# OpenBMB/VisRAG

Measured on NVIDIA H100. Metric: page-images encoded/sec, higher is better.
Workload: dtype bf16

## Files before the change

visrag_b200/csrc/gemm.cu:

```cuda
#include "common.h"
#include "gemm.cuh"

namespace vr {

template <bool F16, int BN, int MODE, bool OUT_F32, bool GELU, bool SWAP = false>
static int launch_gemm(const void* A, int64_t lda, const void* B, int64_t ldb, const GemmArgs& g, cudaStream_t stream) {
    using Cfg = GemmCfg<BN>;
    CUtensorMap ta, tb;
    if (int rc = make_tmap_2d(SWAP ? &tb : &ta, A, g.M, g.K, lda, SWAP ? 64 : GEMM_BM, GEMM_BK, 128, !F16)) return rc;
    if (int rc = make_tmap_2d(SWAP ? &ta : &tb, B, g.N, g.K, ldb, SWAP ? GEMM_BM : 64, GEMM_BK, 128, !F16)) return rc;
    auto kern = gemm_wgmma_kernel<F16, BN, MODE, OUT_F32, GELU, SWAP>;
    static unsigned long long attr_set = 0;
    if (first_use_on_device(&attr_set))
        VR_CHECK_CUDA(cudaFuncSetAttribute(kern, cudaFuncAttributeMaxDynamicSharedMemorySize, Cfg::SMEM_BYTES));
    const int tiles = SWAP ? ((g.N + GEMM_BM - 1) / GEMM_BM) * ((g.M + BN - 1) / BN)
                           : ((g.M + GEMM_BM - 1) / GEMM_BM) * ((g.N + BN - 1) / BN);
    const int grid = tiles < num_sms() ? tiles : num_sms();
    kern<<<grid, GEMM_THREADS, Cfg::SMEM_BYTES, stream>>>(ta, tb, g);
    VR_CHECK_CUDA(cudaGetLastError());
    return 0;
}

template <bool F16, int MODE, bool OUT_F32, bool GELU, int CLUSTER, bool LEAN>
static int launch_pingpong(const void* A, int64_t lda, const void* B, int64_t ldb, const GemmArgs& g, bool l2_slices,
                           cudaStream_t stream) {
    CUtensorMap ta, tb;
    if (int rc = make_tmap_2d(&ta, A, g.M, g.K, lda, GEMM_BM, GEMM_BK, 128, !F16)) return rc;
    if (int rc = make_tmap_2d(&tb, B, g.N, g.K, ldb, 64, GEMM_BK, 128, !F16)) return rc;
    auto kern = gemm_pingpong_kernel<F16, MODE, OUT_F32, GELU, CLUSTER, LEAN>;
    cudaLaunchConfig_t cfg = {};
    cudaLaunchAttribute attr[1];
    cfg.blockDim = dim3(GEMM_THREADS);
    cfg.dynamicSmemBytes = GEMM_PP_SMEM_BYTES;
    cfg.stream = stream;
    attr[0].id = cudaLaunchAttributeClusterDimension;
    attr[0].val.clusterDim.x = CLUSTER;
    attr[0].val.clusterDim.y = 1;
    attr[0].val.clusterDim.z = 1;
    cfg.attrs = attr;
    cfg.numAttrs = 1;
    static unsigned long long attr_set = 0;
    static int max_clusters[64] = {};
    const int dev = current_device(), dev_slot = dev >= 0 && dev < 64 ? dev : 0;
    if (first_use_on_device(&attr_set)) {
        VR_CHECK_CUDA(cudaFuncSetAttribute(kern, cudaFuncAttributeMaxDynamicSharedMemorySize, GEMM_PP_SMEM_BYTES));
        int n = num_sms() / CLUSTER;
        if (CLUSTER > 1) {
            cfg.gridDim = dim3(num_sms() / CLUSTER * CLUSTER);
            VR_CHECK_CUDA(cudaOccupancyMaxActiveClusters(&n, kern, &cfg));
        }
        max_clusters[dev_slot] = n;
    }
    const PPSched sch = pp_schedule(g.M, g.N, g.K, CLUSTER, l2_slices);
    VR_REQUIRE(max_clusters[dev_slot] > 0, "vr_gemm: no %d-CTA cluster of the ping-pong kernel fits on this device", CLUSTER);
    const int units = sch.num_units();
    const int clusters = units < max_clusters[dev_slot] ? units : max_clusters[dev_slot];
    cfg.gridDim = dim3(clusters * CLUSTER);
    VR_CHECK_CUDA(cudaLaunchKernelEx(&cfg, kern, ta, tb, g, sch));
    return 0;
}

template <bool F16>
static int check_out_dtype(const vr_gemm_epilogue& e) {
    if (F16) {
        if (e.mode == VR_EPI_LINEAR && e.out_dtype == VR_F32) {
            VR_REQUIRE(!e.act_gelu, "vr_gemm: GELU epilogue writes fp16 only (fp16 operands)");
            return 0;
        }
        if (e.mode == VR_EPI_LINEAR)
            VR_REQUIRE(e.out_dtype == VR_F16, "vr_gemm: with fp16 operands out_dtype must be VR_F16 or VR_F32");
        else
            VR_REQUIRE(e.out_dtype == VR_F16, "vr_gemm: with fp16 operands ROPE / SWIGLU write fp16: out_dtype must be VR_F16");
        return 0;
    }
    if (e.mode != VR_EPI_LINEAR) return 0;
    if (e.out_dtype == VR_F32) {
        VR_REQUIRE(!e.act_gelu, "vr_gemm: GELU epilogue writes bf16 only");
        return 0;
    }
    VR_REQUIRE(e.out_dtype == VR_BF16, "vr_gemm: out_dtype must be VR_BF16 or VR_F32");
    return 0;
}

template <bool F16>
static int dispatch_swapped(const void* A, int64_t lda, const void* B, int64_t ldb, const GemmArgs& g, cudaStream_t s) {
    const vr_gemm_epilogue& e = g.epi;
    VR_REQUIRE(e.mode == VR_EPI_LINEAR, "vr_gemm: block_n=3 (feature-major accumulator) supports LINEAR epilogues only");
    if (int rc = check_out_dtype<F16>(e)) return rc;
    if (e.out_dtype == VR_F32) return launch_gemm<F16, 128, VR_EPI_LINEAR, true, false, true>(A, lda, B, ldb, g, s);
    if (e.act_gelu) return launch_gemm<F16, 128, VR_EPI_LINEAR, false, true, true>(A, lda, B, ldb, g, s);
    return launch_gemm<F16, 128, VR_EPI_LINEAR, false, false, true>(A, lda, B, ldb, g, s);
}

constexpr int PP = 2, PP_MC = 4, PP_NFAST = 5;
template <bool F16, int BN, int MODE, bool OUT_F32, bool GELU, bool LEAN = false>
static int launch_any(const void* A, int64_t lda, const void* B, int64_t ldb, const GemmArgs& g, cudaStream_t s) {
    if constexpr (BN < 0)
        return launch_pingpong<F16, MODE, OUT_F32, GELU, -BN == PP_MC ? 2 : 1, LEAN>(A, lda, B, ldb, g, -BN != PP_NFAST, s);
    else return launch_gemm<F16, BN, MODE, OUT_F32, GELU>(A, lda, B, ldb, g, s);
}

template <bool F16, int BN>
static int dispatch_mode(const void* A, int64_t lda, const void* B, int64_t ldb, const GemmArgs& g, cudaStream_t s) {
    const vr_gemm_epilogue& e = g.epi;
    switch (e.mode) {
        case VR_EPI_LINEAR: {
            if (int rc = check_out_dtype<F16>(e)) return rc;
            if (e.out_dtype == VR_F32) return launch_any<F16, BN, VR_EPI_LINEAR, true, false>(A, lda, B, ldb, g, s);
            const bool lean = BN < 0 && e.bias && e.scale == 1.0f && !e.rowadd && !e.resid;
            if (e.act_gelu)
                return lean ? launch_any<F16, BN, VR_EPI_LINEAR, false, true, true>(A, lda, B, ldb, g, s)
                            : launch_any<F16, BN, VR_EPI_LINEAR, false, true>(A, lda, B, ldb, g, s);
            return lean ? launch_any<F16, BN, VR_EPI_LINEAR, false, false, true>(A, lda, B, ldb, g, s)
                        : launch_any<F16, BN, VR_EPI_LINEAR, false, false>(A, lda, B, ldb, g, s);
        }
        case VR_EPI_ROPE:
            VR_REQUIRE(e.positions && e.rope_cos && e.rope_sin, "vr_gemm: ROPE epilogue needs positions/cos/sin");
            VR_REQUIRE(g.N % 64 == 0 && e.rope_cols % 64 == 0, "vr_gemm: ROPE needs N and rope_cols multiples of 64");
            if (int rc = check_out_dtype<F16>(e)) return rc;
            return launch_any<F16, BN, VR_EPI_ROPE, false, false>(A, lda, B, ldb, g, s);
        case VR_EPI_SWIGLU:
            VR_REQUIRE(g.N % 64 == 0, "vr_gemm: SWIGLU needs N multiple of 64");
            if (int rc = check_out_dtype<F16>(e)) return rc;
            return launch_any<F16, BN, VR_EPI_SWIGLU, false, false>(A, lda, B, ldb, g, s);
        default:
            set_error("vr_gemm: unknown epilogue mode %d", e.mode);
            return 2;
    }
}

template <bool F16>
static int dispatch_block_n(const void* A, int64_t lda, const void* B, int64_t ldb, const GemmArgs& g, int bn, cudaStream_t s) {
    if (bn == PP) return dispatch_mode<F16, -PP>(A, lda, B, ldb, g, s);
    if (bn == PP_MC) return dispatch_mode<F16, -PP_MC>(A, lda, B, ldb, g, s);
    if (bn == PP_NFAST) return dispatch_mode<F16, -PP_NFAST>(A, lda, B, ldb, g, s);
    if (bn == 3) return dispatch_swapped<F16>(A, lda, B, ldb, g, s);
    if (bn == 256) return dispatch_mode<F16, 256>(A, lda, B, ldb, g, s);
    if (bn == 192) return dispatch_mode<F16, 192>(A, lda, B, ldb, g, s);
    if (bn == 128) return dispatch_mode<F16, 128>(A, lda, B, ldb, g, s);
    if (bn == 64) return dispatch_mode<F16, 64>(A, lda, B, ldb, g, s);
    set_error("vr_gemm: block_n must be 0 (auto), 64, 128, 192, 256, 2 / 4 / 5 (ping-pong) or 3 (feature-major accumulator)");
    return 2;
}

}

extern "C" int vr_gemm_tuned(const void* A, int64_t lda, const void* B, int64_t ldb, int32_t ab_dtype, int32_t M,
                             int32_t N, int32_t K, const vr_gemm_epilogue* epi, int32_t block_n, void* stream) {
    using namespace vr;
    VR_REQUIRE(A && B && epi && epi->out, "vr_gemm: null pointer argument");
    VR_REQUIRE(M > 0 && N > 0 && K > 0, "vr_gemm: empty problem M=%d N=%d K=%d", M, N, K);
    VR_REQUIRE(ab_dtype == VR_BF16 || ab_dtype == VR_F16, "vr_gemm: operands must be bf16 or fp16 (got dtype %d)", ab_dtype);
    VR_REQUIRE(N % 8 == 0, "vr_gemm: N=%d must be a multiple of 8", N);
    VR_REQUIRE(K % 8 == 0, "vr_gemm: K=%d must be a multiple of 8 (16-byte TMA rows)", K);
    const int64_t out_cols = epi->mode == VR_EPI_SWIGLU ? N / 2 : N;
    VR_REQUIRE(epi->ldo >= out_cols && epi->ldo % 8 == 0, "vr_gemm: ldo=%lld too small or not a multiple of 8",
               (long long)epi->ldo);
    VR_REQUIRE(epi->mode != VR_EPI_LINEAR || (reinterpret_cast<uintptr_t>(epi->out) & 15) == 0,
               "vr_gemm: a LINEAR out must be 16-byte aligned (out=%p)", epi->out);
    VR_REQUIRE_ALIGNED("vr_gemm", "A", A, 16);
    VR_REQUIRE_ALIGNED("vr_gemm", "B", B, 16);
    VR_REQUIRE_ALIGNED("vr_gemm", "bias", epi->bias, 8);
    VR_REQUIRE_ALIGNED("vr_gemm", "rowadd", epi->rowadd, 8);
    VR_REQUIRE_ALIGNED("vr_gemm", "resid", epi->resid, 8);
    VR_REQUIRE_ALIGNED("vr_gemm", "rope_cos", epi->rope_cos, 8);
    VR_REQUIRE_ALIGNED("vr_gemm", "rope_sin", epi->rope_sin, 8);
    VR_REQUIRE_ALIGNED("vr_gemm", "positions", epi->positions, 4);
    VR_REQUIRE_ALIGNED("vr_gemm", "out", epi->out, 4);
    GemmArgs g;
    g.M = M; g.N = N; g.K = K; g.epi = *epi;
    cudaStream_t s = reinterpret_cast<cudaStream_t>(stream);
    int bn = block_n;
    if (bn == 0) {
        bn = M <= 128 ? 64 : PP_MC;
    }
    return ab_dtype == VR_F16 ? dispatch_block_n<true>(A, lda, B, ldb, g, bn, s) : dispatch_block_n<false>(A, lda, B, ldb, g, bn, s);
}

extern "C" int vr_gemm(const void* A, int64_t lda, const void* B, int64_t ldb, int32_t ab_dtype, int32_t M, int32_t N,
                       int32_t K, const vr_gemm_epilogue* epi, void* stream) {
    return vr_gemm_tuned(A, lda, B, ldb, ab_dtype, M, N, K, epi, 0, stream);
}
```

visrag_b200/csrc/gemm.cuh:

```cuda
#pragma once
#include "ptx.cuh"
#include "../../include/visrag_b200.h"

namespace vr {

constexpr int GEMM_BM = 128;
constexpr int GEMM_BK = 64;
constexpr int GEMM_THREADS = 3 * 128;

template <int BN>
struct GemmCfg {
    static_assert(BN % 64 == 0 && BN <= 256, "tile width: 64, 128, 192 or 256");
    static constexpr int A_BYTES = GEMM_BM * GEMM_BK * 2;
    static constexpr int B_BYTES = BN * GEMM_BK * 2;
    static constexpr int STAGE_BYTES = A_BYTES + B_BYTES;
    static constexpr int STAGES = (192 * 1024) / STAGE_BYTES;
    static constexpr int SMEM_BYTES = STAGES * STAGE_BYTES + 1024  + 256 ;
};

struct GemmArgs {
    int M, N, K;
    vr_gemm_epilogue epi;
};

__device__ __forceinline__ float erf_as(float x) {
    const float ax = fabsf(x);
    float t;
    asm("rcp.approx.ftz.f32 %0, %1;" : "=f"(t) : "f"(fmaf(0.3275911f, ax, 1.0f)));
    float p = fmaf(1.061405429f, t, -1.453152027f);
    p = fmaf(p, t, 1.421413741f);
    p = fmaf(p, t, -0.284496736f);
    p = fmaf(p, t, 0.254829592f);
    p *= t;
    float e;
    asm("ex2.approx.ftz.f32 %0, %1;" : "=f"(e) : "f"(-1.4426950408889634f * ax * ax));
    return copysignf(fmaf(-p, e, 1.0f), x);
}
__device__ __forceinline__ float gelu_erf(float x) { return 0.5f * x * (1.0f + erf_as(x * 0.70710678118654752f)); }

#ifndef VR_GELU_POLY
#define VR_GELU_POLY 1
#endif
#if VR_GELU_POLY
template <int N>
__device__ __forceinline__ void gelu_erf_n(float (&x)[N]) {
    constexpr float R2 = 0.70710678118654752f, ZMAX = 3.2f, A = 2.0f / (ZMAX * ZMAX);
    constexpr float C[11] = {2.982273671e-03f, -7.046153472e-03f, 7.957076705e-03f, -1.521942819e-02f, 3.318292224e-02f,
                             -5.471928813e-02f, 8.062700147e-02f, -1.136467381e-01f, 1.543549678e-01f, -2.173077339e-01f,
                             4.413341836e-01f};
    float z[N], u[N], p[N];
#pragma unroll
    for (int i = 0; i < N; ++i) z[i] = fminf(fmaxf(x[i] * R2, -ZMAX), ZMAX);
#pragma unroll
    for (int i = 0; i < N; ++i) u[i] = fmaf(fmaf(z[i], z[i], 0.0f), A, -1.0f);
#pragma unroll
    for (int i = 0; i < N; ++i) p[i] = fmaf(u[i], C[0], C[1]);
#pragma unroll
    for (int k = 2; k < 11; ++k) {
#pragma unroll
        for (int i = 0; i < N; ++i) p[i] = fmaf(p[i], u[i], C[k]);
    }
#pragma unroll
    for (int i = 0; i < N; ++i) {
        const float r = fmaf(p[i], z[i], 0.0f);
        const float h = 0.5f * x[i];
        x[i] = fmaf(h, r, h);
    }
}
__device__ __forceinline__ void gelu_erf2(float& x0, float& x1) {
    float x[2] = {x0, x1};
    gelu_erf_n(x);
    x0 = x[0];
    x1 = x[1];
}
#else
__device__ __forceinline__ void pk_fma(float& d0, float& d1, float a0, float a1, float b0, float b1, float c0, float c1) {
    d0 = fmaf(a0, b0, c0);
    d1 = fmaf(a1, b1, c1);
}
__device__ __forceinline__ void gelu_erf2(float& x0, float& x1) {
    constexpr float R2 = 0.70710678118654752f;
    const float a0 = fabsf(x0) * R2, a1 = fabsf(x1) * R2;
    float d0, d1, t0, t1, p0, p1, q0, q1, e0, e1, r0, r1;
    pk_fma(d0, d1, a0, a1, 0.3275911f, 0.3275911f, 1.0f, 1.0f);
    asm("rcp.approx.ftz.f32 %0, %1;" : "=f"(t0) : "f"(d0));
    asm("rcp.approx.ftz.f32 %0, %1;" : "=f"(t1) : "f"(d1));
    pk_fma(p0, p1, t0, t1, 1.061405429f, 1.061405429f, -1.453152027f, -1.453152027f);
    pk_fma(p0, p1, p0, p1, t0, t1, 1.421413741f, 1.421413741f);
    pk_fma(p0, p1, p0, p1, t0, t1, -0.284496736f, -0.284496736f);
    pk_fma(p0, p1, p0, p1, t0, t1, 0.254829592f, 0.254829592f);
    pk_fma(p0, p1, p0, p1, t0, t1, 0.0f, 0.0f);
    pk_fma(q0, q1, a0, a1, a0, a1, 0.0f, 0.0f);
    asm("ex2.approx.ftz.f32 %0, %1;" : "=f"(e0) : "f"(q0 * -1.4426950408889634f));
    asm("ex2.approx.ftz.f32 %0, %1;" : "=f"(e1) : "f"(q1 * -1.4426950408889634f));
    pk_fma(r0, r1, p0, p1, -e0, -e1, 1.0f, 1.0f);
    r0 = copysignf(r0, x0);
    r1 = copysignf(r1, x1);
    const float h0 = 0.5f * x0, h1 = 0.5f * x1;
    pk_fma(x0, x1, h0, h1, r0, r1, h0, h1);
}
template <int N>
__device__ __forceinline__ void gelu_erf_n(float (&x)[N]) {
#pragma unroll
    for (int i = 0; i < N; i += 2) gelu_erf2(x[i], x[i + 1]);
}
#endif
__device__ __forceinline__ float silu(float x) {
    float e, r;
    asm("ex2.approx.ftz.f32 %0, %1;" : "=f"(e) : "f"(x * -1.4426950408889634f));
    asm("rcp.approx.ftz.f32 %0, %1;" : "=f"(r) : "f"(1.0f + e));
    return x * r;
}

template <bool F16, bool OUT_F32, bool GELU>
__device__ __forceinline__ void epi_linear2(const GemmArgs& g, int row, int col, float x0, float x1) {
    const vr_gemm_epilogue& e = g.epi;
    if (row >= g.M || col >= g.N) return;
    if (e.bias) {
        const float2 b = *reinterpret_cast<const float2*>(e.bias + col);
        x0 += b.x; x1 += b.y;
    }
    if (GELU) gelu_erf2(x0, x1);
    if (e.scale != 1.0f) { x0 *= e.scale; x1 *= e.scale; }
    if (e.rowadd) {
        const float2 a2 = *reinterpret_cast<const float2*>(e.rowadd + static_cast<long long>(row % e.rowadd_period) * g.N + col);
        x0 += a2.x; x1 += a2.y;
    }
    const long long o = static_cast<long long>(row) * e.ldo + col;
    if (e.resid) {
        const float2 r2 = *reinterpret_cast<const float2*>(e.resid + o);
        x0 += r2.x; x1 += r2.y;
    }
    if (OUT_F32) *reinterpret_cast<float2*>(reinterpret_cast<float*>(e.out) + o) = make_float2(x0, x1);
    else *reinterpret_cast<uint32_t*>(reinterpret_cast<half16_t<F16>*>(e.out) + o) = pack16x2<F16>(x0, x1);
}

template <bool F16, bool OUT_F32, bool GELU>
__device__ __forceinline__ void epi_linear_t(const GemmArgs& g, int tok, int f, float x) {
    const vr_gemm_epilogue& e = g.epi;
    if (tok >= g.M || f >= g.N) return;
    if (e.bias) x += e.bias[f];
    if (GELU) {
        float y = x;
        gelu_erf2(x, y);
    }
    if (e.scale != 1.0f) x *= e.scale;
    if (e.rowadd) x += e.rowadd[static_cast<long long>(tok % e.rowadd_period) * g.N + f];
    const long long o = static_cast<long long>(tok) * e.ldo + f;
    if (e.resid) x += e.resid[o];
    if (OUT_F32) reinterpret_cast<float*>(e.out)[o] = x;
    else reinterpret_cast<half16_t<F16>*>(e.out)[o] = to_half16<F16>(x);
}

template <bool F16>
__device__ __forceinline__ void epi_rope2(const GemmArgs& g, int row, int head0, int c, float lo0, float lo1, float hi0,
                                          float hi1) {
    const vr_gemm_epilogue& e = g.epi;
    if (row >= g.M || head0 >= g.N) return;
    if (head0 < e.rope_cols) {
        const long long pos = e.positions[row];
        const float2 cs = *reinterpret_cast<const float2*>(e.rope_cos + pos * 32 + c);
        const float2 sn = *reinterpret_cast<const float2*>(e.rope_sin + pos * 32 + c);
        const float a0 = lo0, a1 = lo1, b0 = hi0, b1 = hi1;
        lo0 = a0 * cs.x - b0 * sn.x; hi0 = b0 * cs.x + a0 * sn.x;
        lo1 = a1 * cs.y - b1 * sn.y; hi1 = b1 * cs.y + a1 * sn.y;
    }
    half16_t<F16>* o = reinterpret_cast<half16_t<F16>*>(e.out) + static_cast<long long>(row) * e.ldo + head0 + c;
    *reinterpret_cast<uint32_t*>(o) = pack16x2<F16>(lo0, lo1);
    *reinterpret_cast<uint32_t*>(o + 32) = pack16x2<F16>(hi0, hi1);
}

template <bool F16>
__device__ __forceinline__ void epi_swiglu2(const GemmArgs& g, int row, int blk0, int c, float g0, float g1, float u0, float u1) {
    const vr_gemm_epilogue& e = g.epi;
    if (row >= g.M || blk0 >= g.N) return;
    half16_t<F16>* o = reinterpret_cast<half16_t<F16>*>(e.out) + static_cast<long long>(row) * e.ldo + (blk0 >> 1) + c;
    *reinterpret_cast<uint32_t*>(o) = pack16x2<F16>(silu(g0) * u0, silu(g1) * u1);
}

template <bool F16, int BN, int MODE, bool OUT_F32, bool GELU, bool SWAP = false>
__global__ void __launch_bounds__(GEMM_THREADS, 1)
gemm_wgmma_kernel(const __grid_constant__ CUtensorMap tmap_a, const __grid_constant__ CUtensorMap tmap_b, const GemmArgs g) {
    using Cfg = GemmCfg<BN>;
    constexpr int STAGES = Cfg::STAGES;

    extern __shared__ uint8_t smem_raw[];
    uint8_t* smem = reinterpret_cast<uint8_t*>((reinterpret_cast<uintptr_t>(smem_raw) + 1023) & ~uintptr_t(1023));
    uint8_t* smem_a = smem;
    uint8_t* smem_b = smem + STAGES * Cfg::A_BYTES;
    uint64_t* full_bar = reinterpret_cast<uint64_t*>(smem + STAGES * Cfg::STAGE_BYTES);
    uint64_t* empty_bar = full_bar + STAGES;

    const int wg = threadIdx.x >> 7;
    const int warp = (threadIdx.x >> 5) & 3;
    const int lane = threadIdx.x & 31;

    static_assert(!SWAP || MODE == VR_EPI_LINEAR, "feature-major accumulators are implemented for LINEAR epilogues");
    const int tiles_m = ((SWAP ? g.N : g.M) + GEMM_BM - 1) / GEMM_BM;
    const int tiles_n = ((SWAP ? g.M : g.N) + BN - 1) / BN;
    const int num_tiles = tiles_m * tiles_n;
    const int num_kb = (g.K + GEMM_BK - 1) / GEMM_BK;
    auto tile_m0 = [&](int t) { return (SWAP ? t % tiles_m : t / tiles_n) * GEMM_BM; };
    auto tile_n0 = [&](int t) { return (SWAP ? t / tiles_m : t % tiles_n) * BN; };

    if (threadIdx.x == 0) {
        tma_prefetch_desc(&tmap_a);
        tma_prefetch_desc(&tmap_b);
        for (int i = 0; i < STAGES; ++i) {
            mbar_init(&full_bar[i], 1);
            mbar_init(&empty_bar[i], 8);
        }
        fence_mbar_init();
    }
    __syncthreads();

    if (wg == 0) {
        setmaxnreg_dec<40>();
        if (warp == 0 && lane == 0) {
            int stage = 0;
            uint32_t phase = 0;
            for (int t = blockIdx.x; t < num_tiles; t += gridDim.x) {
                const int m0 = tile_m0(t);
                const int n0 = tile_n0(t);
                for (int kb = 0; kb < num_kb; ++kb) {
                    mbar_wait(&empty_bar[stage], phase ^ 1);
                    mbar_expect_tx(&full_bar[stage], Cfg::STAGE_BYTES);
                    tma_load_2d(&tmap_a, &full_bar[stage], smem_a + stage * Cfg::A_BYTES, kb * GEMM_BK, m0);
#pragma unroll
                    for (int h = 0; h < BN / 64; ++h)
                        tma_load_2d(&tmap_b, &full_bar[stage], smem_b + stage * Cfg::B_BYTES + h * (64 * GEMM_BK * 2),
                                    kb * GEMM_BK, n0 + h * 64);
                    if (++stage == STAGES) { stage = 0; phase ^= 1; }
                }
            }
        }
    } else {
        setmaxnreg_inc<232>();
        const int cw = wg - 1;
        const uint64_t desc_hi = make_smem_desc(0, 16, 1024, kLayoutSW128);
        const uint32_t a_lo0 = (smem_u32(smem_a) + cw * (64 * GEMM_BK * 2)) >> 4, b_lo0 = smem_u32(smem_b) >> 4;
        const int g8 = lane >> 2, q = lane & 3;
        int stage = 0;
        uint32_t phase = 0;
        for (int t = blockIdx.x; t < num_tiles; t += gridDim.x) {
            float acc[BN / 2];
            int prev = -1;
            for (int kb = 0; kb < num_kb; ++kb) {
                mbar_wait(&full_bar[stage], phase);
                const uint64_t ad = desc_hi | static_cast<uint64_t>(a_lo0 + stage * (Cfg::A_BYTES >> 4));
                const uint64_t bd = desc_hi | static_cast<uint64_t>(b_lo0 + stage * (Cfg::B_BYTES >> 4));
                wgmma_fence();
#pragma unroll
                for (int kk = 0; kk < 4; ++kk)
                    wgmma_ss<F16, false>(acc, ad + 2 * kk, bd + 2 * kk, (kb | kk) != 0, std::integral_constant<int, BN>());
                wgmma_commit();
                if (prev >= 0) {
                    wgmma_wait<1>();
                    if (lane == 0) mbar_arrive(&empty_bar[prev]);
                }
                prev = stage;
                if (++stage == STAGES) { stage = 0; phase ^= 1; }
            }
            wgmma_wait<0>();
            if (lane == 0) mbar_arrive(&empty_bar[prev]);
            wgmma_touch(acc);

            const int r0 = tile_m0(t) + cw * 64 + warp * 16 + g8;
            const int n0 = tile_n0(t);
            if (MODE == VR_EPI_LINEAR) {
#pragma unroll
                for (int j = 0; j < BN / 8; ++j) {
                    const int c = n0 + j * 8 + q * 2;
                    if (SWAP) {
                        epi_linear_t<F16, OUT_F32, GELU>(g, c, r0, acc[4 * j]);
                        epi_linear_t<F16, OUT_F32, GELU>(g, c + 1, r0, acc[4 * j + 1]);
                        epi_linear_t<F16, OUT_F32, GELU>(g, c, r0 + 8, acc[4 * j + 2]);
                        epi_linear_t<F16, OUT_F32, GELU>(g, c + 1, r0 + 8, acc[4 * j + 3]);
                    } else {
                        epi_linear2<F16, OUT_F32, GELU>(g, r0, c, acc[4 * j], acc[4 * j + 1]);
                        epi_linear2<F16, OUT_F32, GELU>(g, r0 + 8, c, acc[4 * j + 2], acc[4 * j + 3]);
                    }
                }
            } else {
#pragma unroll
                for (int hb = 0; hb < BN / 64; ++hb) {
#pragma unroll
                    for (int j = 0; j < 4; ++j) {
                        const int lo = 4 * (hb * 8 + j), hi = 4 * (hb * 8 + j + 4);
                        const int blk0 = n0 + hb * 64, c = j * 8 + q * 2;
                        if (MODE == VR_EPI_ROPE) {
                            epi_rope2<F16>(g, r0, blk0, c, acc[lo], acc[lo + 1], acc[hi], acc[hi + 1]);
                            epi_rope2<F16>(g, r0 + 8, blk0, c, acc[lo + 2], acc[lo + 3], acc[hi + 2], acc[hi + 3]);
                        } else {
                            epi_swiglu2<F16>(g, r0, blk0, c, acc[lo], acc[lo + 1], acc[hi], acc[hi + 1]);
                            epi_swiglu2<F16>(g, r0 + 8, blk0, c, acc[lo + 2], acc[lo + 3], acc[hi + 2], acc[hi + 3]);
                        }
                    }
                }
            }
        }
    }
}

constexpr int GEMM_PP_BN = 128;
constexpr int GEMM_PP_A_BYTES = GEMM_BM * GEMM_BK * 2;
constexpr int GEMM_PP_B_BYTES = GEMM_PP_BN * GEMM_BK * 2;
constexpr int GEMM_PP_STAGE_BYTES = GEMM_PP_A_BYTES + GEMM_PP_B_BYTES;
constexpr int GEMM_PP_STAGES = (192 * 1024) / GEMM_PP_STAGE_BYTES;
constexpr int GEMM_PP_SMEM_BYTES = GEMM_PP_STAGES * GEMM_PP_STAGE_BYTES + 1024 + 256 + 2 * GEMM_PP_BN * 4;
constexpr int GEMM_PP_BAR_BIAS = 3;
constexpr int GEMM_PP_BAR_TURN = 1;

constexpr long long GEMM_PP_L2_SLICE = 20ll << 20;

struct PPSched {
    int units_m, tiles_n, slice_w;
    __host__ __device__ int num_units() const { return units_m * tiles_n; }
    __device__ void coords(int u, int& um, int& tn) const {
        const int slice_units = units_m * slice_w;
        const int s = u / slice_units, r = u - s * slice_units;
        const int w = min(slice_w, tiles_n - s * slice_w);
        um = r / w;
        tn = s * slice_w + r % w;
    }
};

inline PPSched pp_schedule(int M, int N, int K, int cluster, bool l2_slices) {
    PPSched s;
    s.units_m = ((M + GEMM_BM - 1) / GEMM_BM + cluster - 1) / cluster;
    s.tiles_n = (N + GEMM_PP_BN - 1) / GEMM_PP_BN;
    s.slice_w = s.tiles_n;
    if (l2_slices) {
        long long fit = GEMM_PP_L2_SLICE / (static_cast<long long>(GEMM_PP_BN) * K * 2);
        if (fit < 1) fit = 1;
        if (fit < s.tiles_n) {
            const int slices = static_cast<int>((s.tiles_n + fit - 1) / fit);
            s.slice_w = (s.tiles_n + slices - 1) / slices;
        }
    }
    return s;
}

__device__ __forceinline__ void quad_transpose4(uint32_t (&w)[4], int q) {
    const bool b1 = q & 2, b0 = q & 1;
    uint32_t r0 = __shfl_xor_sync(0xffffffffu, b1 ? w[0] : w[2], 2);
    uint32_t r1 = __shfl_xor_sync(0xffffffffu, b1 ? w[1] : w[3], 2);
    if (b1) { w[0] = r0; w[1] = r1; } else { w[2] = r0; w[3] = r1; }
    r0 = __shfl_xor_sync(0xffffffffu, b0 ? w[0] : w[1], 1);
    r1 = __shfl_xor_sync(0xffffffffu, b0 ? w[2] : w[3], 1);
    if (b0) { w[0] = r0; w[2] = r1; } else { w[1] = r0; w[3] = r1; }
}

constexpr int PP_EPI_BATCH = 4;
template <bool F16, bool OUT_F32, bool GELU>
__device__ __forceinline__ void pp_epilogue_linear(const GemmArgs& g, const float (&acc)[64], int r0, int n0, int q2) {
    const vr_gemm_epilogue& e = g.epi;
    const bool row_ok[2] = {r0 < g.M, r0 + 8 < g.M};
    const long long o[2] = {static_cast<long long>(r0) * e.ldo, static_cast<long long>(r0 + 8) * e.ldo};
    long long ra[2] = {0, 0};
    if (e.rowadd) {
        ra[0] = static_cast<long long>(r0 % e.rowadd_period) * g.N;
        ra[1] = static_cast<long long>((r0 + 8) % e.rowadd_period) * g.N;
    }
#pragma unroll
    for (int jb = 0; jb < GEMM_PP_BN / 8; jb += PP_EPI_BATCH) {
        float2 bias[PP_EPI_BATCH], add[PP_EPI_BATCH][2], res[PP_EPI_BATCH][2];
#pragma unroll
        for (int j = 0; j < PP_EPI_BATCH; ++j) {
            const int c = n0 + (jb + j) * 8 + q2;
            const bool col_ok = c < g.N;
            bias[j] = make_float2(0.0f, 0.0f);
            if (e.bias && col_ok) bias[j] = __ldg(reinterpret_cast<const float2*>(e.bias + c));
#pragma unroll
            for (int h = 0; h < 2; ++h) {
                add[j][h] = res[j][h] = make_float2(0.0f, 0.0f);
                if (e.rowadd && col_ok && row_ok[h]) add[j][h] = __ldg(reinterpret_cast<const float2*>(e.rowadd + ra[h] + c));
                if (e.resid && col_ok && row_ok[h]) res[j][h] = *reinterpret_cast<const float2*>(e.resid + o[h] + c);
            }
        }
        uint32_t w16[2][PP_EPI_BATCH];
#pragma unroll
        for (int j = 0; j < PP_EPI_BATCH; ++j) {
            const int c = n0 + (jb + j) * 8 + q2;
#pragma unroll
            for (int h = 0; h < 2; ++h) {
                if (OUT_F32 && (!row_ok[h] || c >= g.N)) continue;
                float x0 = acc[4 * (jb + j) + 2 * h], x1 = acc[4 * (jb + j) + 2 * h + 1];
                if (e.bias) { x0 += bias[j].x; x1 += bias[j].y; }
                if (GELU) gelu_erf2(x0, x1);
                if (e.scale != 1.0f) { x0 *= e.scale; x1 *= e.scale; }
                if (e.rowadd) { x0 += add[j][h].x; x1 += add[j][h].y; }
                if (e.resid) { x0 += res[j][h].x; x1 += res[j][h].y; }
                if (OUT_F32) *reinterpret_cast<float2*>(reinterpret_cast<float*>(e.out) + o[h] + c) = make_float2(x0, x1);
                else w16[h][j] = pack16x2<F16>(x0, x1);
            }
        }
        if (!OUT_F32) {
            static_assert(PP_EPI_BATCH == 4, "the quad transpose moves 4 column groups");
            const int q = q2 >> 1, c = n0 + (jb + q) * 8;
#pragma unroll
            for (int h = 0; h < 2; ++h) {
                quad_transpose4(w16[h], q);
                if (row_ok[h] && c < g.N)
                    *reinterpret_cast<uint4*>(reinterpret_cast<half16_t<F16>*>(e.out) + o[h] + c) =
                        make_uint4(w16[h][0], w16[h][1], w16[h][2], w16[h][3]);
            }
        }
    }
}

__device__ __forceinline__ void pp_stage_bias(float* slot, const GemmArgs& g, int n0, int t) {
    if (n0 + t < g.N) cp_async_4(slot + t, g.epi.bias + n0 + t);
}
template <bool F16, bool GELU, bool GUARD>
__device__ __forceinline__ void pp_epilogue_lean(const GemmArgs& g, const float (&acc)[64], const float* bias, int r0, int n0,
                                                 int q) {
    const vr_gemm_epilogue& e = g.epi;
    half16_t<F16>* out = reinterpret_cast<half16_t<F16>*>(e.out) + static_cast<long long>(r0) * e.ldo + n0 + 8 * q;
    const long long row8 = 8 * e.ldo;
    const bool row_ok[2] = {r0 < g.M, r0 + 8 < g.M};
#pragma unroll
    for (int jb = 0; jb < GEMM_PP_BN / 8; jb += 4) {
        float x[16];
#pragma unroll
        for (int j = 0; j < 4; ++j) {
            const float2 b = ld_shared_f2(bias + 8 * (jb + j) + 2 * q);
#pragma unroll
            for (int h = 0; h < 2; ++h) {
                x[4 * j + 2 * h] = acc[4 * (jb + j) + 2 * h] + b.x;
                x[4 * j + 2 * h + 1] = acc[4 * (jb + j) + 2 * h + 1] + b.y;
            }
        }
        if (GELU) gelu_erf_n(x);
        uint32_t w16[2][4];
#pragma unroll
        for (int j = 0; j < 4; ++j) {
#pragma unroll
            for (int h = 0; h < 2; ++h) w16[h][j] = pack16x2<F16>(x[4 * j + 2 * h], x[4 * j + 2 * h + 1]);
        }
#pragma unroll
        for (int h = 0; h < 2; ++h) {
            quad_transpose4(w16[h], q);
            if (!GUARD || (row_ok[h] && n0 + 8 * (jb + q) < g.N))
                *reinterpret_cast<uint4*>(out + h * row8 + 8 * jb) = make_uint4(w16[h][0], w16[h][1], w16[h][2], w16[h][3]);
        }
    }
}

template <bool F16, int MODE, bool OUT_F32, bool GELU>
__device__ __forceinline__ void pp_epilogue(const GemmArgs& g, const float (&acc)[64], int r0, int n0, int q2) {
    if (MODE == VR_EPI_LINEAR) {
        pp_epilogue_linear<F16, OUT_F32, GELU>(g, acc, r0, n0, q2);
    } else {
#pragma unroll
        for (int hb = 0; hb < GEMM_PP_BN / 64; ++hb) {
#pragma unroll
            for (int j = 0; j < 4; ++j) {
                const int lo = 4 * (hb * 8 + j), hi = 4 * (hb * 8 + j + 4);
                const int blk0 = n0 + hb * 64, c = j * 8 + q2;
                if (MODE == VR_EPI_ROPE) {
                    epi_rope2<F16>(g, r0, blk0, c, acc[lo], acc[lo + 1], acc[hi], acc[hi + 1]);
                    epi_rope2<F16>(g, r0 + 8, blk0, c, acc[lo + 2], acc[lo + 3], acc[hi + 2], acc[hi + 3]);
                } else {
                    epi_swiglu2<F16>(g, r0, blk0, c, acc[lo], acc[lo + 1], acc[hi], acc[hi + 1]);
                    epi_swiglu2<F16>(g, r0 + 8, blk0, c, acc[lo + 2], acc[lo + 3], acc[hi + 2], acc[hi + 3]);
                }
            }
        }
    }
}

template <bool F16, int MODE, bool OUT_F32, bool GELU, int CLUSTER, bool LEAN = false>
__global__ void __launch_bounds__(GEMM_THREADS, 1)
gemm_pingpong_kernel(const __grid_constant__ CUtensorMap tmap_a, const __grid_constant__ CUtensorMap tmap_b, const GemmArgs g,
                     const PPSched sch) {
    static_assert(CLUSTER == 1 || CLUSTER == 2, "CTA pairs at most");
    static_assert(!LEAN || (MODE == VR_EPI_LINEAR && !OUT_F32), "the lean epilogue writes 16-bit LINEAR outputs");
    constexpr int STAGES = GEMM_PP_STAGES;
    extern __shared__ uint8_t smem_raw[];
    uint8_t* smem = reinterpret_cast<uint8_t*>((reinterpret_cast<uintptr_t>(smem_raw) + 1023) & ~uintptr_t(1023));
    uint8_t* smem_a = smem;
    uint8_t* smem_b = smem + STAGES * GEMM_PP_A_BYTES;
    uint64_t* full_bar = reinterpret_cast<uint64_t*>(smem + STAGES * GEMM_PP_STAGE_BYTES);
    uint64_t* empty_bar = full_bar + STAGES;
    float* bias_slots = reinterpret_cast<float*>(smem + STAGES * GEMM_PP_STAGE_BYTES + 256);

    const int wg = threadIdx.x >> 7;
    const int warp = (threadIdx.x >> 5) & 3;
    const int lane = threadIdx.x & 31;
    const int num_kb = (g.K + GEMM_BK - 1) / GEMM_BK;
    const int rank = CLUSTER == 1 ? 0 : static_cast<int>(cluster_ctarank());
    const int unit0 = blockIdx.x / CLUSTER, unit_step = gridDim.x / CLUSTER;
    const int num_units = sch.num_units();

    if (threadIdx.x == 0) {
        tma_prefetch_desc(&tmap_a);
        tma_prefetch_desc(&tmap_b);
        for (int i = 0; i < STAGES; ++i) {
            mbar_init(&full_bar[i], 1);
            mbar_init(&empty_bar[i], 4 * CLUSTER);
        }
        fence_mbar_init();
    }
    if (CLUSTER == 1) __syncthreads();
    else cluster_sync_all();

    if (wg == 0) {
        setmaxnreg_dec<40>();
        if (warp == 0 && lane == 0) {
            int stage = 0;
            uint32_t phase = 0;
            for (int u = unit0; u < num_units; u += unit_step) {
                int um, tn;
                sch.coords(u, um, tn);
                const int m0 = (um * CLUSTER + rank) * GEMM_BM, n0 = tn * GEMM_PP_BN;
                for (int kb = 0; kb < num_kb; ++kb) {
                    mbar_wait(&empty_bar[stage], phase ^ 1);
                    mbar_expect_tx(&full_bar[stage], GEMM_PP_STAGE_BYTES);
                    tma_load_2d(&tmap_a, &full_bar[stage], smem_a + stage * GEMM_PP_A_BYTES, kb * GEMM_BK, m0);
                    uint8_t* b_dst = smem_b + stage * GEMM_PP_B_BYTES;
                    if (CLUSTER == 1) {
#pragma unroll
                        for (int h = 0; h < GEMM_PP_BN / 64; ++h)
                            tma_load_2d(&tmap_b, &full_bar[stage], b_dst + h * (64 * GEMM_BK * 2), kb * GEMM_BK, n0 + h * 64);
                    } else {
                        tma_load_2d_multicast(&tmap_b, &full_bar[stage], b_dst + rank * (64 * GEMM_BK * 2), kb * GEMM_BK,
                                              n0 + rank * 64, 0x3);
                    }
                    if (++stage == STAGES) { stage = 0; phase ^= 1; }
                }
            }
        }
    } else {
        setmaxnreg_inc<232>();
        const int me = wg - 1;
        const uint64_t desc_hi = make_smem_desc(0, 16, 1024, kLayoutSW128);
        const uint32_t a_lo0 = smem_u32(smem_a) >> 4, b_lo0 = smem_u32(smem_b) >> 4;
        constexpr uint32_t HALF = (64 * GEMM_BK * 2) >> 4;
        const int g8 = lane >> 2, q = lane & 3;
        float* bias_slot = bias_slots + me * GEMM_PP_BN;
        auto release = [&](int s) {
            if (lane != 0) return;
            if (CLUSTER == 1) {
                mbar_arrive(&empty_bar[s]);
            } else {
#pragma unroll
                for (int r = 0; r < CLUSTER; ++r) mbar_arrive_cluster(&empty_bar[s], r);
            }
        };
        for (int i = me, u = unit0 + me * unit_step; u < num_units; i += 2, u += 2 * unit_step) {
            const int pos = i * num_kb;
            int stage = pos % STAGES;
            uint32_t phase = (pos / STAGES) & 1;
            if (i > 0) named_bar_sync(GEMM_PP_BAR_TURN + me, 256);
            if constexpr (LEAN) {
                int um, tn;
                sch.coords(u, um, tn);
                pp_stage_bias(bias_slot, g, tn * GEMM_PP_BN, threadIdx.x & 127);
            }
            float acc0[64], acc1[64];
            int prev = -1;
            for (int kb = 0; kb < num_kb; ++kb) {
                mbar_wait(&full_bar[stage], phase);
                const uint64_t ad = desc_hi | static_cast<uint64_t>(a_lo0 + stage * (GEMM_PP_A_BYTES >> 4));
                const uint64_t bd = desc_hi | static_cast<uint64_t>(b_lo0 + stage * (GEMM_PP_B_BYTES >> 4));
                wgmma_fence();
#pragma unroll
                for (int kk = 0; kk < 4; ++kk) {
                    wgmma_ss<F16, false>(acc0, ad + 2 * kk, bd + 2 * kk, (kb | kk) != 0, std::integral_constant<int, 128>());
                    wgmma_ss<F16, false>(acc1, ad + HALF + 2 * kk, bd + 2 * kk, (kb | kk) != 0,
                                           std::integral_constant<int, 128>());
                }
                wgmma_commit();
                if (prev >= 0) {
                    wgmma_wait<1>();
                    release(prev);
                }
                prev = stage;
                if (++stage == STAGES) { stage = 0; phase ^= 1; }
            }
            if (u + unit_step < num_units) named_bar_arrive(GEMM_PP_BAR_TURN + (me ^ 1), 256);
            wgmma_wait<0>();
            release(prev);
            wgmma_touch(acc0);
            wgmma_touch(acc1);

            int um, tn;
            sch.coords(u, um, tn);
            const int m0 = (um * CLUSTER + rank) * GEMM_BM, n0 = tn * GEMM_PP_BN;
            if constexpr (LEAN) {
                cp_async_wait_all();
                named_bar_sync(GEMM_PP_BAR_BIAS + me, 128);
                if (m0 + GEMM_BM <= g.M && n0 + GEMM_PP_BN <= g.N) {
                    pp_epilogue_lean<F16, GELU, false>(g, acc0, bias_slot, m0 + warp * 16 + g8, n0, q);
                    pp_epilogue_lean<F16, GELU, false>(g, acc1, bias_slot, m0 + 64 + warp * 16 + g8, n0, q);
                } else {
                    pp_epilogue_lean<F16, GELU, true>(g, acc0, bias_slot, m0 + warp * 16 + g8, n0, q);
                    pp_epilogue_lean<F16, GELU, true>(g, acc1, bias_slot, m0 + 64 + warp * 16 + g8, n0, q);
                }
            } else {
                pp_epilogue<F16, MODE, OUT_F32, GELU>(g, acc0, m0 + warp * 16 + g8, n0, q * 2);
                pp_epilogue<F16, MODE, OUT_F32, GELU>(g, acc1, m0 + 64 + warp * 16 + g8, n0, q * 2);
            }
        }
    }
    if (CLUSTER == 2) cluster_sync_all();
}

}
```

Baseline: 347.6.

## Generalize ping-pong GEMM clusters to 4x1 and 2x2 TMA multicast shapes

```diff
diff --git a/visrag_b200/csrc/gemm.cu b/visrag_b200/csrc/gemm.cu
--- a/visrag_b200/csrc/gemm.cu
+++ b/visrag_b200/csrc/gemm.cu
@@ -21,13 +21,14 @@
     return 0;
 }
 
-template <bool F16, int MODE, bool OUT_F32, bool GELU, int CLUSTER, bool LEAN>
+template <bool F16, int MODE, bool OUT_F32, bool GELU, int CM, int CN, bool LEAN>
 static int launch_pingpong(const void* A, int64_t lda, const void* B, int64_t ldb, const GemmArgs& g, bool l2_slices,
                            cudaStream_t stream) {
+    constexpr int CLUSTER = CM * CN;
     CUtensorMap ta, tb;
-    if (int rc = make_tmap_2d(&ta, A, g.M, g.K, lda, GEMM_BM, GEMM_BK, 128, !F16)) return rc;
-    if (int rc = make_tmap_2d(&tb, B, g.N, g.K, ldb, 64, GEMM_BK, 128, !F16)) return rc;
-    auto kern = gemm_pingpong_kernel<F16, MODE, OUT_F32, GELU, CLUSTER, LEAN>;
+    if (int rc = make_tmap_2d(&ta, A, g.M, g.K, lda, GEMM_BM / CN, GEMM_BK, 128, !F16)) return rc;
+    if (int rc = make_tmap_2d(&tb, B, g.N, g.K, ldb, CM == 1 ? 64 : GEMM_PP_BN / CM, GEMM_BK, 128, !F16)) return rc;
+    auto kern = gemm_pingpong_kernel<F16, MODE, OUT_F32, GELU, CM, CN, LEAN>;
     cudaLaunchConfig_t cfg = {};
     cudaLaunchAttribute attr[1];
     cfg.blockDim = dim3(GEMM_THREADS);
@@ -51,7 +52,7 @@
         }
         max_clusters[dev_slot] = n;
     }
-    const PPSched sch = pp_schedule(g.M, g.N, g.K, CLUSTER, l2_slices);
+    const PPSched sch = pp_schedule(g.M, g.N, g.K, CM, CN, l2_slices);
     VR_REQUIRE(max_clusters[dev_slot] > 0, "vr_gemm: no %d-CTA cluster of the ping-pong kernel fits on this device", CLUSTER);
     const int units = sch.num_units();
     const int clusters = units < max_clusters[dev_slot] ? units : max_clusters[dev_slot];
@@ -92,12 +93,15 @@
     return launch_gemm<F16, 128, VR_EPI_LINEAR, false, false, true>(A, lda, B, ldb, g, s);
 }
 
-constexpr int PP = 2, PP_MC = 4, PP_NFAST = 5;
+constexpr int PP = 2, PP_MC = 4, PP_NFAST = 5, PP_MC41 = 6, PP_MC22 = 7;
 template <bool F16, int BN, int MODE, bool OUT_F32, bool GELU, bool LEAN = false>
 static int launch_any(const void* A, int64_t lda, const void* B, int64_t ldb, const GemmArgs& g, cudaStream_t s) {
-    if constexpr (BN < 0)
-        return launch_pingpong<F16, MODE, OUT_F32, GELU, -BN == PP_MC ? 2 : 1, LEAN>(A, lda, B, ldb, g, -BN != PP_NFAST, s);
-    else return launch_gemm<F16, BN, MODE, OUT_F32, GELU>(A, lda, B, ldb, g, s);
+    if constexpr (BN < 0) {
+        constexpr int CM = -BN == PP_MC || -BN == PP_MC22 ? 2 : -BN == PP_MC41 ? 4 : 1, CN = -BN == PP_MC22 ? 2 : 1;
+        return launch_pingpong<F16, MODE, OUT_F32, GELU, CM, CN, LEAN>(A, lda, B, ldb, g, -BN != PP_NFAST, s);
+    } else {
+        return launch_gemm<F16, BN, MODE, OUT_F32, GELU>(A, lda, B, ldb, g, s);
+    }
 }
 
 template <bool F16, int BN>
@@ -134,12 +138,15 @@
     if (bn == PP) return dispatch_mode<F16, -PP>(A, lda, B, ldb, g, s);
     if (bn == PP_MC) return dispatch_mode<F16, -PP_MC>(A, lda, B, ldb, g, s);
     if (bn == PP_NFAST) return dispatch_mode<F16, -PP_NFAST>(A, lda, B, ldb, g, s);
+    if (bn == PP_MC41) return dispatch_mode<F16, -PP_MC41>(A, lda, B, ldb, g, s);
+    if (bn == PP_MC22) return dispatch_mode<F16, -PP_MC22>(A, lda, B, ldb, g, s);
     if (bn == 3) return dispatch_swapped<F16>(A, lda, B, ldb, g, s);
     if (bn == 256) return dispatch_mode<F16, 256>(A, lda, B, ldb, g, s);
     if (bn == 192) return dispatch_mode<F16, 192>(A, lda, B, ldb, g, s);
     if (bn == 128) return dispatch_mode<F16, 128>(A, lda, B, ldb, g, s);
     if (bn == 64) return dispatch_mode<F16, 64>(A, lda, B, ldb, g, s);
-    set_error("vr_gemm: block_n must be 0 (auto), 64, 128, 192, 256, 2 / 4 / 5 (ping-pong) or 3 (feature-major accumulator)");
+    set_error("vr_gemm: block_n must be 0 (auto), 64, 128, 192, 256, 2 / 4 / 5 / 6 / 7 (ping-pong) or 3 (feature-major "
+              "accumulator)");
     return 2;
 }
 
@@ -172,7 +179,8 @@
     cudaStream_t s = reinterpret_cast<cudaStream_t>(stream);
     int bn = block_n;
     if (bn == 0) {
-        bn = M <= 128 ? 64 : PP_MC;
+        const int tiles_n = (N + GEMM_PP_BN - 1) / GEMM_PP_BN;
+        bn = M <= 128 ? 64 : (tiles_n % 2 == 1 && K >= 4096 && M >= 16384) ? PP_MC41 : PP_MC;
     }
     return ab_dtype == VR_F16 ? dispatch_block_n<true>(A, lda, B, ldb, g, bn, s) : dispatch_block_n<false>(A, lda, B, ldb, g, bn, s);
 }
diff --git a/visrag_b200/csrc/gemm.cuh b/visrag_b200/csrc/gemm.cuh
--- a/visrag_b200/csrc/gemm.cuh
+++ b/visrag_b200/csrc/gemm.cuh
@@ -314,28 +314,28 @@
 constexpr long long GEMM_PP_L2_SLICE = 20ll << 20;
 
 struct PPSched {
-    int units_m, tiles_n, slice_w;
-    __host__ __device__ int num_units() const { return units_m * tiles_n; }
-    __device__ void coords(int u, int& um, int& tn) const {
+    int units_m, units_n, slice_w;
+    __host__ __device__ int num_units() const { return units_m * units_n; }
+    __device__ void coords(int u, int& um, int& un) const {
         const int slice_units = units_m * slice_w;
         const int s = u / slice_units, r = u - s * slice_units;
-        const int w = min(slice_w, tiles_n - s * slice_w);
+        const int w = min(slice_w, units_n - s * slice_w);
         um = r / w;
-        tn = s * slice_w + r % w;
+        un = s * slice_w + r % w;
     }
 };
 
-inline PPSched pp_schedule(int M, int N, int K, int cluster, bool l2_slices) {
+inline PPSched pp_schedule(int M, int N, int K, int cm, int cn, bool l2_slices) {
     PPSched s;
-    s.units_m = ((M + GEMM_BM - 1) / GEMM_BM + cluster - 1) / cluster;
-    s.tiles_n = (N + GEMM_PP_BN - 1) / GEMM_PP_BN;
-    s.slice_w = s.tiles_n;
+    s.units_m = ((M + GEMM_BM - 1) / GEMM_BM + cm - 1) / cm;
+    s.units_n = ((N + GEMM_PP_BN - 1) / GEMM_PP_BN + cn - 1) / cn;
+    s.slice_w = s.units_n;
     if (l2_slices) {
-        long long fit = GEMM_PP_L2_SLICE / (static_cast<long long>(GEMM_PP_BN) * K * 2);
+        long long fit = GEMM_PP_L2_SLICE / (static_cast<long long>(cn) * GEMM_PP_BN * K * 2);
         if (fit < 1) fit = 1;
-        if (fit < s.tiles_n) {
-            const int slices = static_cast<int>((s.tiles_n + fit - 1) / fit);
-            s.slice_w = (s.tiles_n + slices - 1) / slices;
+        if (fit < s.units_n) {
+            const int slices = static_cast<int>((s.units_n + fit - 1) / fit);
+            s.slice_w = (s.units_n + slices - 1) / slices;
         }
     }
     return s;
@@ -470,11 +470,14 @@
     }
 }
 
-template <bool F16, int MODE, bool OUT_F32, bool GELU, int CLUSTER, bool LEAN = false>
+template <bool F16, int MODE, bool OUT_F32, bool GELU, int CM, int CN, bool LEAN = false>
 __global__ void __launch_bounds__(GEMM_THREADS, 1)
 gemm_pingpong_kernel(const __grid_constant__ CUtensorMap tmap_a, const __grid_constant__ CUtensorMap tmap_b, const GemmArgs g,
                      const PPSched sch) {
-    static_assert(CLUSTER == 1 || CLUSTER == 2, "CTA pairs at most");
+    static_assert((CN == 1 && (CM == 1 || CM == 2 || CM == 4)) || (CM == 2 && CN == 2), "1 x 1, 2 x 1, 4 x 1 or 2 x 2 clusters");
+    constexpr int CLUSTER = CM * CN;
+    constexpr int A_ROWS = GEMM_BM / CN, B_ROWS = CM == 1 ? 64 : GEMM_PP_BN / CM;
+    constexpr int PEERS = CM + CN - 1;
     static_assert(!LEAN || (MODE == VR_EPI_LINEAR && !OUT_F32), "the lean epilogue writes 16-bit LINEAR outputs");
     constexpr int STAGES = GEMM_PP_STAGES;
     extern __shared__ uint8_t smem_raw[];
@@ -490,6 +493,7 @@
     const int lane = threadIdx.x & 31;
     const int num_kb = (g.K + GEMM_BK - 1) / GEMM_BK;
     const int rank = CLUSTER == 1 ? 0 : static_cast<int>(cluster_ctarank());
+    const int mi = CN == 1 ? rank : rank % CM, ni = CN == 1 ? 0 : rank / CM;
     const int unit0 = blockIdx.x / CLUSTER, unit_step = gridDim.x / CLUSTER;
     const int num_units = sch.num_units();
 
@@ -498,7 +502,7 @@
         tma_prefetch_desc(&tmap_b);
         for (int i = 0; i < STAGES; ++i) {
             mbar_init(&full_bar[i], 1);
-            mbar_init(&empty_bar[i], 4 * CLUSTER);
+            mbar_init(&empty_bar[i], 4 * PEERS);
         }
         fence_mbar_init();
     }
@@ -510,22 +514,29 @@
         if (warp == 0 && lane == 0) {
             int stage = 0;
             uint32_t phase = 0;
+            const uint16_t b_mask = ((1u << CM) - 1) << (ni * CM), a_mask = CN == 1 ? 1u << mi : 0x5u << mi;
             for (int u = unit0; u < num_units; u += unit_step) {
-                int um, tn;
-                sch.coords(u, um, tn);
-                const int m0 = (um * CLUSTER + rank) * GEMM_BM, n0 = tn * GEMM_PP_BN;
+                int um, un;
+                sch.coords(u, um, un);
+                const int m0 = (um * CM + mi) * GEMM_BM, n0 = (un * CN + ni) * GEMM_PP_BN;
                 for (int kb = 0; kb < num_kb; ++kb) {
                     mbar_wait(&empty_bar[stage], phase ^ 1);
                     mbar_expect_tx(&full_bar[stage], GEMM_PP_STAGE_BYTES);
-                    tma_load_2d(&tmap_a, &full_bar[stage], smem_a + stage * GEMM_PP_A_BYTES, kb * GEMM_BK, m0);
+                    uint8_t* a_dst = smem_a + stage * GEMM_PP_A_BYTES;
+                    if (CN == 1) {
+                        tma_load_2d(&tmap_a, &full_bar[stage], a_dst, kb * GEMM_BK, m0);
+                    } else {
+                        tma_load_2d_multicast(&tmap_a, &full_bar[stage], a_dst + ni * (A_ROWS * GEMM_BK * 2), kb * GEMM_BK,
+                                              m0 + ni * A_ROWS, a_mask);
+                    }
                     uint8_t* b_dst = smem_b + stage * GEMM_PP_B_BYTES;
-                    if (CLUSTER == 1) {
+                    if (CM == 1) {
 #pragma unroll
                         for (int h = 0; h < GEMM_PP_BN / 64; ++h)
                             tma_load_2d(&tmap_b, &full_bar[stage], b_dst + h * (64 * GEMM_BK * 2), kb * GEMM_BK, n0 + h * 64);
                     } else {
-                        tma_load_2d_multicast(&tmap_b, &full_bar[stage], b_dst + rank * (64 * GEMM_BK * 2), kb * GEMM_BK,
-                                              n0 + rank * 64, 0x3);
+                        tma_load_2d_multicast(&tmap_b, &full_bar[stage], b_dst + mi * (B_ROWS * GEMM_BK * 2), kb * GEMM_BK,
+                                              n0 + mi * B_ROWS, b_mask);
                     }
                     if (++stage == STAGES) { stage = 0; phase ^= 1; }
                 }
@@ -545,7 +556,10 @@
                 mbar_arrive(&empty_bar[s]);
             } else {
 #pragma unroll
-                for (int r = 0; r < CLUSTER; ++r) mbar_arrive_cluster(&empty_bar[s], r);
+                for (int j = 0; j < CM; ++j) mbar_arrive_cluster(&empty_bar[s], ni * CM + j);
+#pragma unroll
+                for (int k = 0; k < CN; ++k)
+                    if (k != ni) mbar_arrive_cluster(&empty_bar[s], mi + k * CM);
             }
         };
         for (int i = me, u = unit0 + me * unit_step; u < num_units; i += 2, u += 2 * unit_step) {
@@ -554,9 +568,9 @@
             uint32_t phase = (pos / STAGES) & 1;
             if (i > 0) named_bar_sync(GEMM_PP_BAR_TURN + me, 256);
             if constexpr (LEAN) {
-                int um, tn;
-                sch.coords(u, um, tn);
-                pp_stage_bias(bias_slot, g, tn * GEMM_PP_BN, threadIdx.x & 127);
+                int um, un;
+                sch.coords(u, um, un);
+                pp_stage_bias(bias_slot, g, (un * CN + ni) * GEMM_PP_BN, threadIdx.x & 127);
             }
             float acc0[64], acc1[64];
             int prev = -1;
@@ -585,9 +599,9 @@
             wgmma_touch(acc0);
             wgmma_touch(acc1);
 
-            int um, tn;
-            sch.coords(u, um, tn);
-            const int m0 = (um * CLUSTER + rank) * GEMM_BM, n0 = tn * GEMM_PP_BN;
+            int um, un;
+            sch.coords(u, um, un);
+            const int m0 = (um * CM + mi) * GEMM_BM, n0 = (un * CN + ni) * GEMM_PP_BN;
             if constexpr (LEAN) {
                 cp_async_wait_all();
                 named_bar_sync(GEMM_PP_BAR_BIAS + me, 128);
@@ -604,7 +618,7 @@
             }
         }
     }
-    if (CLUSTER == 2) cluster_sync_all();
-}
-
-}
+    if (CLUSTER > 1) cluster_sync_all();
+}
+
+}
```

Result: no change. 350.6 (median of 6 runs) (+0.9%).
